# rokulkarni15/distributed-llm-training-inference

Measured on AMD Instinct MI355X. Metric: train tok/s Llama-2-7B ZeRO-3+LoRA at 1/2/4/8 GPUs; serve tok/s + p50 TTFT, higher is better.
Workload: dtype bf16

## Files before the change

### lumen/csrc/kernels/flash_attn.hip

```cpp
#include "common.h"
#include <cstdlib>

namespace lumen {
namespace fa {

typedef __bf16 bf16x8 __attribute__((ext_vector_type(8)));
typedef _Float16 f16x8 __attribute__((ext_vector_type(8)));
typedef float f32x4 __attribute__((ext_vector_type(4)));
typedef short s16x4 __attribute__((ext_vector_type(4)));
typedef __attribute__((address_space(3))) s16x4 lds_s16x4;

constexpr int D = 128;
constexpr int BN = 64;
constexpr int IMG = BN * D * 2;

template <typename T> struct Mfma;
template <> struct Mfma<bf16> {
  static __device__ __forceinline__ f32x4 run(uint4 a, uint4 b, f32x4 c) {
    return __builtin_amdgcn_mfma_f32_16x16x32_bf16(__builtin_bit_cast(bf16x8, a),
                                                   __builtin_bit_cast(bf16x8, b), c, 0, 0, 0);
  }
};
template <> struct Mfma<fp16> {
  static __device__ __forceinline__ f32x4 run(uint4 a, uint4 b, f32x4 c) {
    return __builtin_amdgcn_mfma_f32_16x16x32_f16(__builtin_bit_cast(f16x8, a),
                                                  __builtin_bit_cast(f16x8, b), c, 0, 0, 0);
  }
};

__device__ __forceinline__ int swz(int row) { return ((row & 3) << 2) | ((row >> 2) & 3); }
__device__ __forceinline__ int img_off(int row, int chunk) {
  return row * 256 + ((chunk ^ swz(row)) << 4);
}
template <int SW>
__device__ __forceinline__ int swz_t(int row) {
  if constexpr (SW == 0) return swz(row);
  else return ((row & 1) << 3) | ((row & 2) << 1) | ((row & 4) >> 1);
}
__device__ __forceinline__ unsigned lds_off_g(const char* p) {
  return static_cast<unsigned>(
      reinterpret_cast<uintptr_t>((__attribute__((address_space(3))) const char*)(p)));
}
template <int SW>
__device__ __forceinline__ int img_off_t(int row, int chunk) {
  return row * 256 + ((chunk ^ swz_t<SW>(row)) << 4);
}

template <typename T>
__device__ __forceinline__ void stage64(char* img, const T* base, long long ld, int r0, int rmax) {
#pragma unroll
  for (int i = 0; i < 4; ++i) {
    const int idx = threadIdx.x + i * 256;
    const int row = idx >> 4, ch = idx & 15;
    uint4 v = make_uint4(0, 0, 0, 0);
    if (r0 + row < rmax) v = *reinterpret_cast<const uint4*>(base + (long long)(r0 + row) * ld + ch * 8);
    *reinterpret_cast<uint4*>(img + img_off(row, ch)) = v;
  }
}

template <typename T, int SW = 0>
__device__ __forceinline__ void stage64_async(char* img, const T* base, long long ld, int r0,
                                              int rmax) {
  const int lane = threadIdx.x & 63, wid = threadIdx.x >> 6;
#pragma unroll
  for (int i = 0; i < 4; ++i) {
    const int row = (wid * 4 + i) * 4 + (lane >> 4);
    const int ch = (lane & 15) ^ swz_t<SW>(row);
    int gr = r0 + row;
    gr = gr < rmax ? gr : rmax - 1;
    __builtin_amdgcn_global_load_lds(
        (const void*)(base + (long long)gr * ld + ch * 8),
        (__attribute__((address_space(3))) void*)(img + (wid * 4 + i) * 1024), 16, 0, 0);
  }
}

template <typename T>
__device__ __forceinline__ void stage64_async_s(char* img, const T* base, long long ld, int r0,
                                                int rmax) {
  const int lane = threadIdx.x & 63, wid = __builtin_amdgcn_readfirstlane(threadIdx.x >> 6);
  const char* tile = reinterpret_cast<const char*>(base + (long long)r0 * ld);
  const int last = rmax - 1 - r0;
#pragma unroll
  for (int i = 0; i < 4; ++i) {
    const int row = (wid * 4 + i) * 4 + (lane >> 4);
    const int ch = (lane & 15) ^ swz(row);
    const unsigned off = (unsigned)((row < last ? row : last) * (int)ld + ch * 8) * sizeof(T);
    __builtin_amdgcn_global_load_lds(
        (const void*)(tile + off),
        (__attribute__((address_space(3))) void*)(img + (wid * 4 + i) * 1024), 16, 0, 0);
  }
}

__device__ __forceinline__ void dma16_o(const void* g, const char* lds_wave_base) {
  const unsigned m0 = __builtin_amdgcn_readfirstlane(lds_off_g(lds_wave_base));
  asm volatile("s_mov_b32 m0, %1\n\ts_nop 0\n\tglobal_load_lds_dwordx4 %0, off"
               :: "v"(g), "s"(m0) : "memory", "m0");
}
__device__ __forceinline__ void dma4_o(const void* g, const char* lds_wave_base) {
  const unsigned m0 = __builtin_amdgcn_readfirstlane(lds_off_g(lds_wave_base));
  asm volatile("s_mov_b32 m0, %1\n\ts_nop 0\n\tglobal_load_lds_dword %0, off"
               :: "v"(g), "s"(m0) : "memory", "m0");
}
template <typename T, int SW>
__device__ __forceinline__ void stage64_async_o(char* img, const T* base, long long ld, int r0,
                                                int rmax) {
  const int lane = threadIdx.x & 63, wid = __builtin_amdgcn_readfirstlane(threadIdx.x >> 6);
#pragma unroll
  for (int i = 0; i < 4; ++i) {
    const int row = (wid * 4 + i) * 4 + (lane >> 4);
    const int ch = (lane & 15) ^ swz_t<SW>(row);
    int gr = r0 + row;
    gr = gr < rmax ? gr : rmax - 1;
    dma16_o(base + (long long)gr * ld + ch * 8, img + (wid * 4 + i) * 1024);
  }
}

template <typename T, int SW>
__device__ __forceinline__ void stage64_async8_o(char* img, const T* base, long long ld, int r0,
                                                 int rmax) {
  const int lane = threadIdx.x & 63, wid = threadIdx.x >> 6;
#pragma unroll
  for (int i = 0; i < 2; ++i) {
    const int row = (wid * 2 + i) * 4 + (lane >> 4);
    const int ch = (lane & 15) ^ swz_t<SW>(row);
    int gr = r0 + row;
    gr = gr < rmax ? gr : rmax - 1;
    dma16_o(base + (long long)gr * ld + ch * 8, img + (wid * 2 + i) * 1024);
  }
}

template <typename T>
__device__ __forceinline__ void stage64_paged(char* img, const T* cache, int kvh, int nkv,
                                              const int* bt, int bs, int r0, int rmax) {
  const int lane = threadIdx.x & 63, wid = threadIdx.x >> 6;
#pragma unroll
  for (int i = 0; i < 4; ++i) {
    const int row = (wid * 4 + i) * 4 + (lane >> 4);
    const int ch = (lane & 15) ^ swz(row);
    int gr = r0 + row;
    gr = gr < rmax ? gr : rmax - 1;
    const long long blk = bt[gr / bs];
    const T* src = cache + ((blk * nkv + kvh) * bs + gr % bs) * D + ch * 8;
    __builtin_amdgcn_global_load_lds(
        (const void*)src, (__attribute__((address_space(3))) void*)(img + (wid * 4 + i) * 1024),
        16, 0, 0);
  }
}

__device__ __forceinline__ void wait_vm_all() { __builtin_amdgcn_s_waitcnt(0xF70); }
__device__ __forceinline__ void wait_vm_8() { __builtin_amdgcn_s_waitcnt(0xF78); }
__device__ __forceinline__ void lds_fence_barrier() {
  asm volatile("s_waitcnt lgkmcnt(0)" ::: "memory");
  __builtin_amdgcn_s_barrier();
  asm volatile("" ::: "memory");
}

template <int SW = 0>
__device__ __forceinline__ uint4 row_read(const char* img, int row, int chunk) {
  return *reinterpret_cast<const uint4*>(img + img_off_t<SW>(row, chunk));
}

__device__ __forceinline__ uint2 tr_read_raw(const char* p) {
  s16x4 r = __builtin_amdgcn_ds_read_tr16_b64_v4i16((lds_s16x4*)(p));
  return __builtin_bit_cast(uint2, r);
}

__device__ __forceinline__ uint4 tr_read_img(const char* img, int k0, int n0, int lane) {
  const int L = lane & 15, g = lane >> 4;
  const int col = n0 + 4 * (L & 3);
  const int ch = col >> 3, half = (col >> 2) & 1;
  const int r = k0 + 8 * g + (L >> 2);
  const uint2 lo = tr_read_raw(img + img_off(r, ch) + 8 * half);
  const uint2 hi = tr_read_raw(img + img_off(r + 4, ch) + 8 * half);
  return make_uint4(lo.x, lo.y, hi.x, hi.y);
}

__device__ __forceinline__ uint4 tr_read_y(const char* y, int cols, int k0, int m0, int lane) {
  const int L = lane & 15, g = lane >> 4;
  const int r = k0 + 8 * g + (L >> 2);
  const int c = m0 + 4 * (L & 3);
  const int ld = cols + 4;
  const uint2 lo = tr_read_raw(y + (r * ld + c) * 2);
  const uint2 hi = tr_read_raw(y + ((r + 4) * ld + c) * 2);
  return make_uint4(lo.x, lo.y, hi.x, hi.y);
}

template <typename T>
__device__ __forceinline__ void y_store(char* y, int cols, int k0, int m0, int lane, float v0,
                                        float v1, float v2, float v3) {
  T t[4] = {from_f32<T>(v0), from_f32<T>(v1), from_f32<T>(v2), from_f32<T>(v3)};
  *reinterpret_cast<uint2*>(y + ((k0 + (lane & 15)) * (cols + 4) + m0 + 4 * (lane >> 4)) * 2) =
      *reinterpret_cast<uint2*>(t);
}

template <typename T>
__device__ __forceinline__ uint4 gload16(const T* p, bool ok) {
  return ok ? *reinterpret_cast<const uint4*>(p) : make_uint4(0, 0, 0, 0);
}

template <int CTRL>
__device__ __forceinline__ float dpp(float v) {
  return __builtin_bit_cast(float, __builtin_amdgcn_update_dpp(0, __builtin_bit_cast(int, v), CTRL,
                                                               0xF, 0xF, false));
}
__device__ __forceinline__ float red16_max(float v) {
  v = fmaxf(v, dpp<0xB1>(v));
  v = fmaxf(v, dpp<0x4E>(v));
  v = fmaxf(v, dpp<0x141>(v));
  v = fmaxf(v, dpp<0x140>(v));
  return v;
}
__device__ __forceinline__ float red16_sum(float v) {
  v += dpp<0xB1>(v);
  v += dpp<0x4E>(v);
  v += dpp<0x141>(v);
  v += dpp<0x140>(v);
  return v;
}

__device__ __forceinline__ float fexp2(float x) { return __builtin_amdgcn_exp2f(x); }

struct Args {
  const void* q; const void* k; const void* v;
  long long ldq, ldk, ldv;
  void* o; long long ldo;
  float* lse;
  const int* cu;
  const int* tiles;
  int nh, nkv, T;
  float scale, scale_log2;
  const void* dout; long long lddo;
  void* dq; void* dk; void* dv; long long lddq, lddk, lddv;
  const float* delta;
  const int* rope_pos;
  const float* rope_cos;
  const float* rope_sin;
  const int* kv_lens;
  const int* block_tables;
// ... 910 lines not shown
```

### lumen/csrc/kernels/lora_v3.hip

```cpp
#include "tile128.h"
#include "det.h"

namespace lumen {
namespace lv3 {

using namespace tile;

struct Drop {
  unsigned int seed, thresh;
  float scale;
  long long ld;
  long long col0;
};

__device__ __forceinline__ uint4 mask8(uint4 u, uint32_t keep) {
  const auto wm = [keep](int w) {
    return ((keep >> (2 * w)) & 1u ? 0x0000FFFFu : 0u) | ((keep >> (2 * w + 1)) & 1u ? 0xFFFF0000u : 0u);
  };
  return make_uint4(u.x & wm(0), u.y & wm(1), u.z & wm(2), u.w & wm(3));
}

template <typename T>
__device__ __forceinline__ uint4 ld_f32x8(const float* p, bool ok) {
  if (!ok) return make_uint4(0, 0, 0, 0);
  const float4 u = *reinterpret_cast<const float4*>(p);
  const float4 v = *reinterpret_cast<const float4*>(p + 4);
  return make_uint4(pk2<T>(u.x, u.y), pk2<T>(u.z, u.w), pk2<T>(v.x, v.y), pk2<T>(v.z, v.w));
}

struct DownArgs {
  const void* x; long long ldx;
  const float* A; long long lda;
  float* Z; long long ldz;
  int T, K;
  float alpha;
  Drop drop;
  int probe;
  void* xe; long long ldxe; int xk, KP;
  unsigned* cnt;
  float* slab;
};

template <typename T, bool DROP, int NJ>
__global__ void __launch_bounds__(512) down3_kernel(DownArgs a) {
  constexpr int J = NJ * 16, JP = J + 4;
  __shared__ float red[4][64 * JP];
  const int wid = threadIdx.x >> 6, lane = threadIdx.x & 63, L = lane & 15, g = lane >> 4;
  const int t0 = blockIdx.x * 64;
  const int k0 = (blockIdx.y * 8 + wid) * 128;
  f32x4 acc[4][NJ];
#pragma unroll
  for (int rt = 0; rt < 4; ++rt)
#pragma unroll
    for (int jt = 0; jt < NJ; ++jt) acc[rt][jt] = f32x4{0.f, 0.f, 0.f, 0.f};
  if (k0 < a.K) {
    const T* x = reinterpret_cast<const T*>(a.x);
    uint4 xv[4][4];
#pragma unroll
    for (int rt = 0; rt < 4; ++rt)
#pragma unroll
      for (int i = 0; i < 4; ++i) {
        const int t = t0 + rt * 16 + L, c = k0 + 32 * i + 8 * g;
        xv[rt][i] = (t < a.T && c < a.K)
                        ? *reinterpret_cast<const uint4*>(x + (long long)t * a.ldx + c)
                        : make_uint4(0, 0, 0, 0);
      }
    float4 af[4][NJ][2];
    if (!(a.probe & 2)) {
#pragma unroll
      for (int i = 0; i < 4; ++i) {
        const int c = min(k0 + 32 * i + 8 * g, a.K - 8);
#pragma unroll
        for (int jt = 0; jt < NJ; ++jt) {
          const float* ap = a.A + (long long)(jt * 16 + L) * a.lda + c;
          af[i][jt][0] = *reinterpret_cast<const float4*>(ap);
          af[i][jt][1] = *reinterpret_cast<const float4*>(ap + 4);
        }
      }
    }
    if (DROP && !(a.probe & 1)) {
#pragma unroll
      for (int rt = 0; rt < 4; ++rt)
#pragma unroll
// ... 216 lines not shown
    if (rt + 1 < kUpRT && t0 + 16 < a.T) load_tile(t0 + 16, bnxt, ynxt);
    f32x4 acc[8];
#pragma unroll
    for (int n = 0; n < 8; ++n) acc[n] = f32x4{0.f, 0.f, 0.f, 0.f};
#pragma unroll
    for (int ks = 0; ks < NKS; ++ks)
#pragma unroll
      for (int n = 0; n < 8; ++n) acc[n] = Mfma<T>::run(aop[n][ks], bcur[ks], acc[n]);
    const int t = t0 + L;
    float y[4][8];
#pragma unroll
    for (int i = 0; i < 4; ++i) {
      unpack8<T>(ycur[i], y[i]);
      const int c = c0 + 32 * i + 8 * g;
      const uint32_t keep = DROP ? dropout_keep8(a.drop.seed,
                                                 (unsigned long long)((long long)t * a.drop.ld + a.drop.col0 + a.seg.out_off[seg] + c),
                                                 a.drop.thresh)
                                 : 0xFFu;
      const float sc = DROP ? a.alpha * a.drop.scale : a.alpha;
#pragma unroll
      for (int e = 0; e < 8; ++e) {
        const float d = acc[2 * i + (e >> 2)][e & 3];
        y[i][e] += ((keep >> e) & 1u) ? sc * d : 0.f;
      }
    }
    if (rope && t < a.T) {
      const long long p = (long long)a.rope_pos[t] * 64;
      float cs[2][8], sn[2][8];
#pragma unroll
      for (int h = 0; h < 2; ++h) {
        const float* cp = a.rope_cos + p + 32 * h + 8 * g;
        const float* sp = a.rope_sin + p + 32 * h + 8 * g;
        const float4 c_lo = *reinterpret_cast<const float4*>(cp), c_hi = *reinterpret_cast<const float4*>(cp + 4);
        const float4 s_lo = *reinterpret_cast<const float4*>(sp), s_hi = *reinterpret_cast<const float4*>(sp + 4);
        cs[h][0] = c_lo.x; cs[h][1] = c_lo.y; cs[h][2] = c_lo.z; cs[h][3] = c_lo.w;
        cs[h][4] = c_hi.x; cs[h][5] = c_hi.y; cs[h][6] = c_hi.z; cs[h][7] = c_hi.w;
        sn[h][0] = s_lo.x; sn[h][1] = s_lo.y; sn[h][2] = s_lo.z; sn[h][3] = s_lo.w;
        sn[h][4] = s_hi.x; sn[h][5] = s_hi.y; sn[h][6] = s_hi.z; sn[h][7] = s_hi.w;
      }
#pragma unroll
      for (int i = 0; i < 2; ++i)
#pragma unroll
        for (int e = 0; e < 8; ++e) {
          const float lo = y[i][e], hi = y[i + 2][e];
          y[i][e] = lo * cs[i][e] - hi * sn[i][e];
          y[i + 2][e] = hi * cs[i][e] + lo * sn[i][e];
        }
    }
    if (t < a.T) {
#pragma unroll
      for (int i = 0; i < 4; ++i) {
        const int c = c0 + 32 * i + 8 * g;
        if (c < NC) store8(out + (long long)t * a.ldo + c, y[i]);
      }
    }
#pragma unroll
    for (int ks = 0; ks < NKS; ++ks) bcur[ks] = bnxt[ks];
#pragma unroll
    for (int i = 0; i < 4; ++i) ycur[i] = ynxt[i];
  }
}

struct DySeg {
  long long n_off[4], r_off[4], b_off[4];
  int n_len[4];
  int nseg;
};

struct DyArgs {
  const void* dy; long long ldy;
  const float* B; int r;
  const float* Z; long long ldz;
  float* dZ; long long lddz;
  float* dB;
  int T, TW;
  float alpha;
  DySeg seg;
  int probe;
  float* slab_z; float* slab_b;
  unsigned* cnt_z; unsigned* cnt_b;
};

constexpr int kDyCC = 2;

template <typename T>
__device__ __forceinline__ void dy_load(uint4 (&v)[4], const T* base, long long ld, int r0, int rmax,
                                        int c0, int cmax) {
#pragma unroll
  for (int i = 0; i < 4; ++i) {
    const int idx = threadIdx.x + i * 256;
    const int r = r0 + (idx >> 4), c = c0 + (idx & 15) * 8;
    const uint4 u = *reinterpret_cast<const uint4*>(base + (long long)min(r, rmax - 1) * ld +
                                                     min(c, cmax - 8));
    v[i] = (r < rmax && c < cmax) ? u : make_uint4(0, 0, 0, 0);
  }
}

__device__ __forceinline__ void dy_store(char* img, const uint4 (&v)[4]) {
#pragma unroll
  for (int i = 0; i < 4; ++i) {
    const int idx = threadIdx.x + i * 256;
    *reinterpret_cast<uint4*>(img + img_off_b(idx >> 4, idx & 15)) = v[i];
  }
}

template <typename T, int NJ>
__global__ void __launch_bounds__(256) dy3_kernel(DyArgs a) {
  __shared__ __attribute__((aligned(16))) char img[2][64 * 256];
  const int seg = blockIdx.z;
  const int NL = a.seg.n_len[seg];
  const int cb = blockIdx.x * 128 * kDyCC;
  const int tb = blockIdx.y * a.TW, te = min(a.T, tb + a.TW);
  if (cb >= NL || tb >= a.T) return;
  const int lane = threadIdx.x & 63, wid = threadIdx.x >> 6, L = lane & 15, g = lane >> 4;
  const T* dy = reinterpret_cast<const T*>(a.dy) + a.seg.n_off[seg];
  const float* B = a.B + a.seg.b_off[seg] * a.r;
  const float* Z = a.Z + a.seg.r_off[seg];
  float* dZ = a.dZ + a.seg.r_off[seg];
  float* dB = a.dB + a.seg.b_off[seg] * a.r;
  const int nch = min(kDyCC, (NL - cb + 127) / 128);

  uint4 bop[kDyCC][4][NJ];
#pragma unroll
  for (int cc = 0; cc < kDyCC; ++cc)
#pragma unroll
    for (int i = 0; i < 4; ++i)
#pragma unroll
      for (int jt = 0; jt < NJ; ++jt) {
        float f[8];
#pragma unroll
        for (int e = 0; e < 8; ++e) {
          const int c = cb + cc * 128 + 32 * i + 8 * g + e;
          const float u = B[(long long)min(c, NL - 1) * a.r + jt * 16 + L];
          f[e] = c < NL ? u : 0.f;
        }
        bop[cc][i][jt] = pack8<T>(f);
      }
  f32x4 dbacc[kDyCC][2][NJ];
#pragma unroll
  for (int cc = 0; cc < kDyCC; ++cc)
#pragma unroll
    for (int m = 0; m < 2; ++m)
#pragma unroll
      for (int jt = 0; jt < NJ; ++jt) dbacc[cc][m][jt] = f32x4{0.f, 0.f, 0.f, 0.f};

  const int nsub = (te - tb + 63) / 64;
  const int nstage = nsub * nch;
  uint4 v[4];
  dy_load<T>(v, dy, a.ldy, tb, te, cb, NL);
  int buf = 0;
  f32x4 dzacc[NJ];
  uint4 zop[2][NJ];
  for (int s = 0; s < nstage; ++s, buf ^= 1) {
    const int ts = s / nch, cc = s % nch;
    const int t0 = tb + ts * 64, cbase = cb + cc * 128;
    dy_store(img[buf], v);
    __syncthreads();
    float zf[2][NJ][8];
#pragma unroll
    for (int ks = 0; ks < 2; ++ks)
#pragma unroll
      for (int jt = 0; jt < NJ; ++jt)
#pragma unroll
        for (int e = 0; e < 8; ++e) {
          const int t = t0 + 32 * ks + 8 * g + e;
          zf[ks][jt][e] = Z[(long long)min(t, te - 1) * a.ldz + jt * 16 + L];
        }
    {
      const int s1 = min(s + 1, nstage - 1);
      const int ts1 = s1 / nch, cc1 = s1 % nch;
      dy_load<T>(v, dy, a.ldy, tb + ts1 * 64, te, cb + cc1 * 128, NL);
    }
    if (cc == 0) {
#pragma unroll
      for (int jt = 0; jt < NJ; ++jt) dzacc[jt] = f32x4{0.f, 0.f, 0.f, 0.f};
    }
    const char* im = img[buf];
#pragma unroll
    for (int i = 0; i < 4; ++i) {
      const uint4 av = row_read_b(im, wid * 16 + L, i * 4 + g);
#pragma unroll
      for (int c2 = 0; c2 < kDyCC; ++c2)
        if (c2 == cc) {
#pragma unroll
          for (int jt = 0; jt < NJ; ++jt) dzacc[jt] = Mfma<T>::run(av, bop[c2][i][jt], dzacc[jt]);
        }
    }
#pragma unroll
    for (int ks = 0; ks < 2; ++ks)
#pragma unroll
      for (int jt = 0; jt < NJ; ++jt) {
        float f[8];
#pragma unroll
        for (int e = 0; e < 8; ++e) f[e] = t0 + 32 * ks + 8 * g + e < te ? zf[ks][jt][e] : 0.f;
        zop[ks][jt] = pack8<T>(f);
      }
#pragma unroll
    for (int ks = 0; ks < 2; ++ks)
#pragma unroll
      for (int m = 0; m < 2; ++m) {
        const uint4 tv = tr_read_img_b(im, ks * 32, wid * 32 + m * 16, lane);
#pragma unroll
        for (int c2 = 0; c2 < kDyCC; ++c2)
          if (c2 == cc) {
#pragma unroll
            for (int jt = 0; jt < NJ; ++jt) dbacc[c2][m][jt] = Mfma<T>::run(tv, zop[ks][jt], dbacc[c2][m][jt]);
          }
      }
    if (cc == nch - 1) {
      if (a.slab_z != nullptr) {
        float* sz = a.slab_z + (((long long)seg * gridDim.y + blockIdx.y) * gridDim.x + blockIdx.x) *
                                   ((long long)a.TW * a.r);
#pragma unroll
        for (int jt = 0; jt < NJ; ++jt)
#pragma unroll
          for (int r = 0; r < 4; ++r) {
            const int t = t0 + wid * 16 + g * 4 + r;
            if (t < te) det::st_wt(sz + (long long)(t - tb) * a.r + jt * 16 + L, dzacc[jt][r]);
          }
      } else {
#pragma unroll
        for (int jt = 0; jt < NJ; ++jt)
#pragma unroll
          for (int r = 0; r < 4; ++r) {
            const int t = t0 + wid * 16 + g * 4 + r;
            if (t < te && (!(a.probe & 16) || dzacc[jt][r] == 1234.5f))
              atomicAdd(dZ + (long long)t * a.lddz + jt * 16 + L, a.alpha * dzacc[jt][r]);
          }
      }
    }
  }
  if (a.slab_z != nullptr) {
    float* sb = a.slab_b + (((long long)seg * gridDim.x + blockIdx.x) * gridDim.y + blockIdx.y) *
                               (256LL * a.r);
#pragma unroll
    for (int cc = 0; cc < kDyCC; ++cc) {
      if (cc >= nch) break;
#pragma unroll
      for (int m = 0; m < 2; ++m)
#pragma unroll
        for (int jt = 0; jt < NJ; ++jt)
#pragma unroll
          for (int r = 0; r < 4; ++r) {
            const int cl = cc * 128 + wid * 32 + m * 16 + g * 4 + r;
            if (cb + cl < NL) det::st_wt(sb + (long long)cl * a.r + jt * 16 + L, dbacc[cc][m][jt][r]);
          }
    }
    if (a.cnt_z == nullptr) return;
    __shared__ int lastf;
    const int ncb = (NL + 128 * kDyCC - 1) / (128 * kDyCC);
    const int J = NJ * 16;
    if (det::last_arriver(a.cnt_z + (long long)seg * gridDim.y + blockIdx.y, ncb, &lastf)) {
      const float* base = a.slab_z + ((long long)seg * gridDim.y + blockIdx.y) * gridDim.x *
                                         ((long long)a.TW * a.r);
      for (int i = threadIdx.x; i < (te - tb) * (J / 2); i += 256) {
        const int tl = i / (J / 2), j = (i % (J / 2)) * 2;
        const float2 v = det::sum_pairs(base + (long long)tl * a.r + j, (long long)a.TW * a.r, ncb);
        float* o = dZ + (long long)(tb + tl) * a.lddz + j;
        o[0] = a.alpha * v.x;
        o[1] = a.alpha * v.y;
      }
    }
    if (det::last_arriver(a.cnt_b + (long long)seg * gridDim.x + blockIdx.x, gridDim.y, &lastf)) {
      const float* base = a.slab_b + ((long long)seg * gridDim.x + blockIdx.x) * gridDim.y *
                                         (256LL * a.r);
      const int nc = min(256, NL - cb);
      for (int i = threadIdx.x; i < nc * (J / 2); i += 256) {
        const int cl = i / (J / 2), j = (i % (J / 2)) * 2;
        const float2 v = det::sum_pairs(base + (long long)cl * a.r + j, 256LL * a.r, gridDim.y);
        float* o = dB + (long long)(cb + cl) * a.r + j;
        o[0] += a.alpha * v.x;
        o[1] += a.alpha * v.y;
      }
    }
    return;
  }
#pragma unroll
  for (int cc = 0; cc < kDyCC; ++cc) {
    if (cc >= nch) break;
#pragma unroll
    for (int m = 0; m < 2; ++m)
#pragma unroll
      for (int jt = 0; jt < NJ; ++jt) {
#pragma unroll
        for (int r = 0; r < 4; ++r) {
          const int c = cb + cc * 128 + wid * 32 + m * 16 + g * 4 + r;
          if (c < NL && (!(a.probe & 32) || dbacc[cc][m][jt][r] == 1234.5f))
            atomicAdd(dB + (long long)c * a.r + jt * 16 + L, a.alpha * dbacc[cc][m][jt][r]);
        }
      }
  }
}

__device__ __forceinline__ float2 sum_pairs_plain(const float* base, long long stride, int n) {
  float2 v = make_float2(0.f, 0.f);
  for (int q0 = 0; q0 < n; q0 += 16) {
    float2 u[16];
#pragma unroll
    for (int k = 0; k < 16; ++k) {
      const int q = q0 + k < n ? q0 + k : n - 1;
      u[k] = *reinterpret_cast<const float2*>(base + q * stride);
    }
#pragma unroll
    for (int k = 0; k < 16; ++k)
      if (q0 + k < n) {
        v.x += u[k].x;
        v.y += u[k].y;
      }
  }
  return v;
}

__global__ void __launch_bounds__(256) dy3_reduce_kernel(DyArgs a, int gx_n, int gy_n) {
  const int seg = blockIdx.y;
  const int NL = a.seg.n_len[seg];
  const int hr = a.r / 2;
  const long long i = (long long)blockIdx.x * 256 + threadIdx.x;
  const int j = (int)(i % hr) * 2;
  if (blockIdx.z == 0) {
    const long long t = i / hr;
    if (t >= a.T) return;
    const int gy = (int)(t / a.TW), tl = (int)(t % a.TW);
    const int ncb = (NL + 128 * kDyCC - 1) / (128 * kDyCC);
    const float* base = a.slab_z + (((long long)seg * gy_n + gy) * gx_n) * ((long long)a.TW * a.r) +
                        (long long)tl * a.r + j;
    const float2 v = sum_pairs_plain(base, (long long)a.TW * a.r, ncb);
    float* o = a.dZ + a.seg.r_off[seg] + t * a.lddz + j;
    o[0] = a.alpha * v.x;
    o[1] = a.alpha * v.y;
  } else {
    const long long c = i / hr;
    if (c >= NL) return;
    const int gx = (int)(c / (128 * kDyCC)), cl = (int)(c % (128 * kDyCC));
    const float* base = a.slab_b + (((long long)seg * gx_n + gx) * gy_n) * (256LL * a.r) +
                        (long long)cl * a.r + j;
    const float2 v = sum_pairs_plain(base, 256LL * a.r, gy_n);
    float* o = a.dB + (a.seg.b_off[seg] + c) * a.r + j;
    o[0] += a.alpha * v.x;
    o[1] += a.alpha * v.y;
  }
}

__global__ void __launch_bounds__(256) dxa3_reduce_kernel(const float* __restrict__ slab,
                                                          float* __restrict__ dA, long long ldda,
                                                          int R, int K, int gy_n, float scale) {
  const long long i = (long long)blockIdx.x * 256 + threadIdx.x;
// ... 378 lines not shown
    default: LV3_DOWN(TT, 4); break;                                                             \
  }
  if (dtype == kBF16) { LV3_DOWN_NJ(bf16) }
  else if (dtype == kF16) { LV3_DOWN_NJ(fp16) }
  else return hipErrorInvalidValue;
#undef LV3_DOWN_NJ
#undef LV3_DOWN
  if (slab != nullptr && cnt == nullptr) {
    const long long n = (long long)T * (R / 2);
    hipLaunchKernelGGL(lv3::down3_reduce_kernel, dim3((unsigned)((n + 255) / 256)), dim3(256), 0,
                       st, (const float*)slab, Z, ldz, T, R, (int)grid.y);
  }
  return hipGetLastError();
}

extern "C" hipError_t lumen_lora3_up(int dtype, int fwd, void* out, long long ldo, const float* s1,
                                     long long ld1, const float* s2, long long ld2, int T, int J,
                                     float alpha, unsigned long long seed, unsigned int thresh,
                                     float drop_scale, long long drop_ld, long long drop_col0,
                                     int nseg, const long long* out_off, const long long* s1_off,
                                     const long long* s2_off, const int* ncols,
                                     const float* rope_cos, const float* rope_sin,
                                     const int* rope_pos, int rope_mask, hipStream_t st) {
  if (T <= 0 || J < 1 || J > 64 || nseg < 1 || nseg > 4 || (ldo & 7) || (ld1 & 3) || (ld2 & 3))
    return hipErrorInvalidValue;
  lv3::UpArgs a;
  a.out = out; a.ldo = ldo; a.s1 = s1; a.ld1 = ld1; a.s2 = s2; a.ld2 = ld2; a.T = T; a.J = J;
  a.alpha = alpha;
  a.drop = {static_cast<unsigned>(seed) ^ static_cast<unsigned>(seed >> 32), thresh, drop_scale,
            drop_ld, drop_col0};
  a.seg.nseg = nseg;
  int maxc = 0;
  for (int i = 0; i < 4; ++i) {
    const bool v = i < nseg;
    a.seg.out_off[i] = v ? out_off[i] : 0; a.seg.s1_off[i] = v ? s1_off[i] : 0;
    a.seg.s2_off[i] = v ? s2_off[i] : 0; a.seg.ncols[i] = v ? ncols[i] : 0;
    if (v && ((ncols[i] & 7) || (out_off[i] & 7) || (s1_off[i] & 3))) return hipErrorInvalidValue;
    if (v && ncols[i] > maxc) maxc = ncols[i];
  }
  a.rope_cos = rope_cos; a.rope_sin = rope_sin; a.rope_pos = rope_pos;
  a.rope_mask = (fwd && rope_cos && rope_sin && rope_pos) ? rope_mask : 0;
  for (int i = 0; i < nseg; ++i)
    if (((a.rope_mask >> i) & 1) && ((out_off[i] & 127) || (ncols[i] & 127))) return hipErrorInvalidValue;
  if (maxc == 0) return hipSuccess;
  const dim3 grid((maxc + 127) / 128, (T + 64 * lv3::kUpRT - 1) / (64 * lv3::kUpRT), nseg), block(256);
  const bool drop = !fwd && thresh != 0;
#define LV3_UP(TT, KJ)                                                                             \
  do {                                                                                           \
    if (fwd) hipLaunchKernelGGL((lv3::up3_kernel<TT, true, false, KJ>), grid, block, 0, st, a);   \
    else if (drop) hipLaunchKernelGGL((lv3::up3_kernel<TT, false, true, KJ>), grid, block, 0, st, a); \
    else hipLaunchKernelGGL((lv3::up3_kernel<TT, false, false, KJ>), grid, block, 0, st, a);     \
  } while (0)
  if (dtype == kBF16) { if (J <= 32) LV3_UP(bf16, 32); else LV3_UP(bf16, 64); }
  else if (dtype == kF16) { if (J <= 32) LV3_UP(fp16, 32); else LV3_UP(fp16, 64); }
  else return hipErrorInvalidValue;
#undef LV3_UP
  return hipGetLastError();
}

extern "C" hipError_t lumen_lora3_dy(int dtype, const void* dy, long long ldy, const float* B, int r,
                                     const float* Z, long long ldz, float* dZ, long long lddz,
                                     float* dB, int T, int tw, float alpha, int nseg,
                                     const long long* n_off, const long long* r_off,
                                     const long long* b_off, const int* n_len, float* slab_z,
                                     float* slab_b, unsigned* cnt_z, unsigned* cnt_b,
                                     hipStream_t st) {
  if (T <= 0 || nseg < 1 || nseg > 4 || (r != 16 && r != 32 && r != 64) || tw < 64 || (tw & 63) ||
      (ldy & 7))
    return hipErrorInvalidValue;
  lv3::DyArgs a;
  a.probe = lv3_probe();
  a.dy = dy; a.ldy = ldy; a.B = B; a.r = r; a.Z = Z; a.ldz = ldz; a.dZ = dZ; a.lddz = lddz;
  a.dB = dB; a.T = T; a.TW = tw; a.alpha = alpha;
  a.slab_z = slab_z; a.slab_b = slab_b; a.cnt_z = cnt_z; a.cnt_b = cnt_b;
  if (slab_z != nullptr && (slab_b == nullptr || (cnt_z == nullptr) != (cnt_b == nullptr) ||
                            (lddz & 1)))
    return hipErrorInvalidValue;
  a.seg.nseg = nseg;
  int maxl = 0;
  for (int i = 0; i < 4; ++i) {
    const bool v = i < nseg;
    a.seg.n_off[i] = v ? n_off[i] : 0; a.seg.r_off[i] = v ? r_off[i] : 0;
    a.seg.b_off[i] = v ? b_off[i] : 0; a.seg.n_len[i] = v ? n_len[i] : 0;
    if (v && ((n_len[i] & 7) || (n_off[i] & 7))) return hipErrorInvalidValue;
    if (v && n_len[i] > maxl) maxl = n_len[i];
  }
  if (maxl == 0) return hipSuccess;
  const dim3 grid((maxl + 128 * lv3::kDyCC - 1) / (128 * lv3::kDyCC), (T + tw - 1) / tw, nseg), block(256);
#define LV3_DY(TT)                                                                                 \
  switch (r) {                                                                                   \
    case 16: hipLaunchKernelGGL((lv3::dy3_kernel<TT, 1>), grid, block, 0, st, a); break;          \
    case 32: hipLaunchKernelGGL((lv3::dy3_kernel<TT, 2>), grid, block, 0, st, a); break;          \
    default: hipLaunchKernelGGL((lv3::dy3_kernel<TT, 4>), grid, block, 0, st, a); break;          \
  }
  if (dtype == kBF16) { LV3_DY(bf16) }
  else if (dtype == kF16) { LV3_DY(fp16) }
  else return hipErrorInvalidValue;
#undef LV3_DY
  if (slab_z != nullptr && cnt_z == nullptr) {
    const long long n = (long long)(T > maxl ? T : maxl) * (r / 2);
    const dim3 rgrid((unsigned)((n + 255) / 256), nseg, 2);
    hipLaunchKernelGGL(lv3::dy3_reduce_kernel, rgrid, dim3(256), 0, st, a, (int)grid.x,
                       (int)grid.y);
  }
  return hipGetLastError();
}

extern "C" hipError_t lumen_lora3_z_tail(int dtype, const float* Z, int R, void* xe, long long ldx,
                                         int K, int KP, int T, hipStream_t st) {
  if (T <= 0) return hipSuccess;
  if ((KP & 7) || R > KP || (ldx & 7) || (K & 7)) return hipErrorInvalidValue;
  const long long n = static_cast<long long>(T) * (KP / 8);
  const dim3 grid(static_cast<unsigned>((n + 255) / 256)), block(256);
  if (dtype == kBF16) hipLaunchKernelGGL(lv3::z_tail_kernel<bf16>, grid, block, 0, st, Z, R, (bf16*)xe, ldx, K, KP, T);
  else if (dtype == kF16) hipLaunchKernelGGL(lv3::z_tail_kernel<fp16>, grid, block, 0, st, Z, R, (fp16*)xe, ldx, K, KP, T);
  else return hipErrorInvalidValue;
  return hipGetLastError();
}

extern "C" hipError_t lumen_lora3_w_tail(int dtype, void* w, long long ldw, int K, const float* B,
                                         int r, int nseg, const long long* n_off,
                                         const long long* b_off, const int* n_len,
                                         const int* r_off, float scale, hipStream_t st) {
  if (nseg < 1 || nseg > 4 || (r & 7) || (ldw & 7) || (K & 7)) return hipErrorInvalidValue;
  lv3::TailSeg sg;
  sg.nseg = nseg;
  int maxn = 0;
  for (int i = 0; i < 4; ++i) {
    const bool v = i < nseg;
    sg.n_off[i] = v ? n_off[i] : 0; sg.b_off[i] = v ? b_off[i] : 0;
    sg.n_len[i] = v ? n_len[i] : 0; sg.r_off[i] = v ? r_off[i] : 0;
    if (v && (r_off[i] & 7)) return hipErrorInvalidValue;
    if (v && n_len[i] > maxn) maxn = n_len[i];
  }
  if (maxn == 0) return hipSuccess;
  const long long n = static_cast<long long>(maxn) * (r / 8);
  const dim3 grid(static_cast<unsigned>((n + 255) / 256), nseg), block(256);
  if (dtype == kBF16) hipLaunchKernelGGL(lv3::w_tail_kernel<bf16>, grid, block, 0, st, (bf16*)w, ldw, K, B, r, sg, scale);
  else if (dtype == kF16) hipLaunchKernelGGL(lv3::w_tail_kernel<fp16>, grid, block, 0, st, (fp16*)w, ldw, K, B, r, sg, scale);
  else return hipErrorInvalidValue;
  return hipGetLastError();
}

extern "C" hipError_t lumen_lora3_dxa(int dtype, const void* x, long long ldx, void* dx,
                                      long long lddx, const float* dZ, const float* A,
                                      long long lda, float* dA, long long ldda, int T, int K,
                                      int R, int tw, unsigned long long seed, unsigned int thresh,
                                      float drop_scale, long long drop_ld, long long drop_col0,
                                      float* delta, float* slab, unsigned* cnt, hipStream_t st) {
  if (T <= 0 || K <= 0 || R < 16 || R > 64 || (R & 15) || (K & 7) || (ldx & 7) || (lddx & 7) ||
      (lda & 3) || tw < 64 || (tw & 63))
    return hipErrorInvalidValue;
  if (delta != nullptr && ((K & 127) || R != 16)) return hipErrorInvalidValue;
  lv3::DxaArgs a;
  a.probe = lv3_probe();
  a.x = x; a.ldx = ldx; a.dx = dx; a.lddx = lddx; a.dZ = dZ; a.A = A; a.lda = lda; a.dA = dA;
  a.ldda = ldda; a.T = T; a.K = K; a.R = R; a.TW = tw; a.delta = delta;
  a.slab = slab; a.cnt = cnt;
  if (slab != nullptr && (ldda & 1)) return hipErrorInvalidValue;
  const bool drop = thresh != 0;
  a.da_scale = drop ? drop_scale : 1.f;
  a.dx_scale = drop ? drop_scale : 1.f;
  a.drop = {static_cast<unsigned>(seed) ^ static_cast<unsigned>(seed >> 32), thresh, drop_scale,
            drop_ld, drop_col0};
  const dim3 grid((K + 127) / 128, (T + tw - 1) / tw), block(256);
#define LV3_DXA(TT, NJ)                                                                            \
  do {                                                                                           \
    if (drop) hipLaunchKernelGGL((lv3::dxa3_kernel<TT, true, NJ>), grid, block, 0, st, a);      \
    else hipLaunchKernelGGL((lv3::dxa3_kernel<TT, false, NJ>), grid, block, 0, st, a);          \
// ... 31 lines not shown
```

### lumen/ops/lora.py

```python
from __future__ import annotations

import math
from typing import List, Optional, Sequence, Tuple

import torch
import torch.nn.functional as F

from ._native import DTYPE_CODE, native, use_native
from .gemm import mm_nt

Seg = Tuple[int, int, int, int]

_M32 = 0xFFFFFFFF


def _lowbias32(x):
    x = x ^ (x >> 16)
    x = (x * 0x7FEB352D) & _M32
    x = x ^ (x >> 15)
    x = (x * 0x846CA68B) & _M32
    x = x ^ (x >> 16)
    return x


# ... 108 lines not shown


def arena_reset(device) -> None:
    if USE_ARENA and device.type == "cuda":
        ARENA.reset(device)


def _zeros(*shape, device, train: bool = False):
    if USE_ARENA and device.type == "cuda" and (train or _IN_BACKWARD[0]):
        return ARENA.zeros(*shape, device=device)
    return torch.zeros(*shape, device=device, dtype=torch.float32)


USE_V3 = _os.environ.get("LUMEN_LORA_V3", "1") != "0"
DY_TW = int(_os.environ.get("LUMEN_LORA_DY_TW", "0"))
DXA_TW = int(_os.environ.get("LUMEN_LORA_DXA_TW", "0"))
DET_SPLIT = _os.environ.get("LUMEN_DET_SPLIT", "1") != "0"
DXA = _os.environ.get("LUMEN_LORA_DXA", "1") != "0"
DELTA_HANDOFF = _os.environ.get("LUMEN_FA_DELTA_HANDOFF", "1") != "0"
_DELTA_SLOT = [None]


DETERMINISTIC = _os.environ.get("LUMEN_LORA_DETERMINISTIC", "0") == "1"
_det: dict = {}


def _det_ws(dev, nfloat: int, ncnt: int):
    key = (str(dev), torch.cuda.current_stream(dev).cuda_stream)
    got = _det.get(key)
    if got is None or got[0].numel() < nfloat or got[1].numel() < ncnt:
        nf = max(nfloat, got[0].numel() if got is not None else 0, 1 << 20)
        nc = max(ncnt, got[1].numel() if got is not None else 0, 4096)
        got = (torch.empty(nf, dtype=torch.float32, device=dev),
               torch.zeros(nc, dtype=torch.int32, device=dev))
        _det[key] = got
    return got


def _v3_ok(r: int, R: int, segs, *mats) -> bool:
    return (USE_V3 and r in (16, 32, 64) and R % 16 == 0 and R <= 64
            and all(s[0] % 8 == 0 and s[1] % 8 == 0 for s in segs)
            and all(m.stride(1) == 1 and m.stride(0) % 8 == 0 for m in mats))


def _lora3_down(x2d, A, Z, p, seed):
    T, K = x2d.shape
    R = A.shape[0]
    cnt = slab = None
    if DETERMINISTIC and x2d.is_cuda:
        slab, cnt = _det_ws(x2d.device, math.ceil(T / 64) * math.ceil(K / 1024) * 64 * R,
                            math.ceil(T / 64))
    native().lora3_down(x2d, x2d.stride(0), A, Z, R, T, K, R, 1.0, int(seed) & 0x7FFFFFFFFFFFFFFF,
                        drop_threshold(p), 1.0 / (1.0 - p) if p > 0 else 1.0, K, 0,
                        None, 0, 0, None if (slab is not None and DET_SPLIT) else cnt, slab)


def _lora3_fwd(x2d, y, A, B, Z, segs, r, scale, p, seed, rope):
    _lora3_down(x2d, A, Z, p, seed)
    fuse = rope is not None and len(segs) <= 4 and _rope_covered(segs, rope[3])
    for i in range(0, len(segs), 4):
        ch = segs[i:i + 4]
        mask = sum(1 << j for j, sg in enumerate(ch) if sg[0] + sg[1] <= rope[3]) if fuse else 0
        _lora2(2, 1, B, Z, y, y.stride(0), 1, scale, T=x2d.shape[0], J=r, split=1,
               segs4=[(b_off * r, r_off, n_off, n_len) for (n_off, n_len, r_off, b_off) in ch],
               rope=(rope[1], rope[2], rope[0], mask) if fuse else None)
    return y, fuse


FOLD = _os.environ.get("LUMEN_LORA_FOLD", "1") != "0"
FOLD_KP = 64


def fold_operand(x2d: torch.Tensor, K: int) -> Optional[torch.Tensor]:
    if (x2d.dim() == 2 and x2d.shape[1] == K and x2d.stride(1) == 1
            and x2d.stride(0) == K + FOLD_KP and x2d.is_cuda):
        return x2d.as_strided((x2d.shape[0], K + FOLD_KP), (K + FOLD_KP, 1))
    return None


def _dy_tw(segs, T: int) -> int:
    if DY_TW:
        return DY_TW
    cols = sum(math.ceil(s[1] / 256) for s in segs)
    return 256 if cols * math.ceil(T / 256) >= 512 else 128


def lora_fwd_native(x2d, y, A, B, segs: Sequence[Seg], r, scale, p, seed, train: bool = False,
                    rope=None):
    T, K = x2d.shape
    R = A.shape[0]
    v3 = (_v3_ok(r, R, segs, x2d, y) and K % 8 == 0
          and A.is_contiguous() and B.is_contiguous() and A.dtype == B.dtype == torch.float32)
    Ntot = y.shape[1]
    act = DTYPE_CODE[x2d.dtype]
    Z = _zeros(T, R, device=x2d.device, train=train)
    if v3:
        y, fuse = _lora3_fwd(x2d, y, A, B, Z, segs, r, scale, p, seed, rope)
        return Z, fuse
    if _v2_ok(r, R, x2d):
        _lora2(0, 1, x2d, A, Z, R, 1, 1.0, T, R, _split(math.ceil(T / 64), K, 256),
               [(0, 0, 0, K)], seed, p, K)
    else:
        _lora_gemm(act, 1, x2d, A, Z, K, K, R, 1, 1.0, [(0, 0, 0, T, R, K)],
                   _ksplit(T, R, K, _bn(R)), seed, p, K)
    if _v2_ok(r, R, x2d, y) and all(s[0] % 8 == 0 and s[1] % 8 == 0 for s in segs):
        fuse = rope is not None and len(segs) <= 4 and _rope_covered(segs, rope[3])
        for i in range(0, len(segs), 4):
            ch = segs[i:i + 4]
            rp = None
            if fuse:
                mask = sum(1 << j for j, sg in enumerate(ch) if sg[0] + sg[1] <= rope[3])
                rp = (rope[1], rope[2], rope[0], mask)
            _lora2(2, 1, B, Z, y, y.stride(0), 1, scale, T, r, 1,
                   [(b_off * r, r_off, n_off, n_len) for (n_off, n_len, r_off, b_off) in ch],
                   rope=rp)
        return Z, fuse
    segs6 = [(r_off, b_off * r, n_off, T, n_len, r) for (n_off, n_len, r_off, b_off) in segs]
    for i in range(0, len(segs6), 4):
        _lora_gemm(act, 6, Z, B, y, R, r, Ntot, 1, scale, segs6[i:i + 4], 1)
    return Z, False


def _rope_covered(segs, ncols: int) -> bool:
    cov = sorted((s[0], s[0] + s[1]) for s in segs if s[0] < ncols)
    cur = 0
    for a, b in cov:
        if a != cur or b > ncols or a % 128 or b % 128:
            return False
        cur = b
    return cur == ncols


def lora_bwd_native(dy, x2d, A, B, Z, dx, segs: Sequence[Seg], r, scale, p, seed,
                    need_dA=True, need_dB=True, dx_fn=None):
    T, K = x2d.shape
    R = A.shape[0]
    Ntot = dy.shape[1]
    act = DTYPE_CODE[dy.dtype]
    dev = dy.device
    v2 = _v2_ok(r, R, x2d, dy)
    v3 = (v2 and _v3_ok(r, R, segs, x2d, dy) and K % 8 == 0 and A.is_contiguous()
          and B.is_contiguous() and A.dtype == B.dtype == torch.float32)
    v3 = v3 and (dx is None or _v3_ok(r, R, segs, dx))
    direct = v2 and DIRECT_GRAD and _direct_ok(A) and _direct_ok(B)
    if v3:
        return _lora3_bwd(dy, x2d, A, B, Z, dx, segs, r, scale, p, seed, need_dA, need_dB, direct,
                          dx_fn)
    if dx_fn is not None:
        dx = dx_fn()
    nA = R * K if need_dA and not direct else 0
    nB = B.shape[0] * r if need_dB and not direct else 0
    ws = _zeros(T * R + nA + nB, device=dev)
    dZ = ws[:T * R].view(T, R)
    if v2:
        for i in range(0, len(segs), 4):
            ch = segs[i:i + 4]
            _lora2(0, 0, dy, B, dZ, R, 1, scale, T, r,
                   _split(math.ceil(T / 64) * len(ch), max(s[1] for s in ch), 256),
                   [(n_off, b_off * r, r_off, n_len) for (n_off, n_len, r_off, b_off) in ch])
    else:
        s2 = [(n_off, b_off * r, r_off, T, r, n_len) for (n_off, n_len, r_off, b_off) in segs]
        for i in range(0, len(s2), 4):
            chunk = s2[i:i + 4]
            _lora_gemm(act, 2, dy, B, dZ, Ntot, r, R, 1, scale, chunk,
                       _ksplit(T, r, max(s[5] for s in chunk), 16, len(chunk)))
    dA = dB = None
    if need_dA:
# ... 302 lines not shown
```

Baseline: 45680.

## Pipeline LoRA dY kernel with LDS DMA ring and staged Z/B transposes

Rewrites the LoRA backward dy3 kernel to stage dY tiles through a 4-deep LDS ring filled by global_load_lds DMA with vmcnt-based waits, replacing the register double buffer. Z and B are now loaded with vectorized float4 reads, packed into a swizzled transposed LDS buffer once per 512-row superblock, and read back as MFMA operands, instead of scalar per-element gathers on every stage. The token-window heuristic is widened to pick tiles of up to 512 rows while keeping at least a minimum block count. Shared DMA helpers move into a common header and now save and restore m0. The larger LDS footprint may lower occupancy, and new alignment checks reject some inputs.

```diff
diff --git a/lumen/csrc/kernels/flash_attn.hip b/lumen/csrc/kernels/flash_attn.hip
--- a/lumen/csrc/kernels/flash_attn.hip
+++ b/lumen/csrc/kernels/flash_attn.hip
@@ -1,8 +1,14 @@
 #include "common.h"
+#include "lds_dma.h"
 #include <cstdlib>
 
 namespace lumen {
 namespace fa {
+
+using tile::dma16_o;
+using tile::dma4_o;
+using tile::lds_fence_barrier;
+using tile::lds_off_g;
 
 typedef __bf16 bf16x8 __attribute__((ext_vector_type(8)));
 typedef _Float16 f16x8 __attribute__((ext_vector_type(8)));
@@ -36,10 +42,6 @@
 __device__ __forceinline__ int swz_t(int row) {
   if constexpr (SW == 0) return swz(row);
   else return ((row & 1) << 3) | ((row & 2) << 1) | ((row & 4) >> 1);
-}
-__device__ __forceinline__ unsigned lds_off_g(const char* p) {
-  return static_cast<unsigned>(
-      reinterpret_cast<uintptr_t>((__attribute__((address_space(3))) const char*)(p)));
 }
 template <int SW>
 __device__ __forceinline__ int img_off_t(int row, int chunk) {
@@ -91,16 +93,6 @@
   }
 }
 
-__device__ __forceinline__ void dma16_o(const void* g, const char* lds_wave_base) {
-  const unsigned m0 = __builtin_amdgcn_readfirstlane(lds_off_g(lds_wave_base));
-  asm volatile("s_mov_b32 m0, %1\n\ts_nop 0\n\tglobal_load_lds_dwordx4 %0, off"
-               :: "v"(g), "s"(m0) : "memory", "m0");
-}
-__device__ __forceinline__ void dma4_o(const void* g, const char* lds_wave_base) {
-  const unsigned m0 = __builtin_amdgcn_readfirstlane(lds_off_g(lds_wave_base));
-  asm volatile("s_mov_b32 m0, %1\n\ts_nop 0\n\tglobal_load_lds_dword %0, off"
-               :: "v"(g), "s"(m0) : "memory", "m0");
-}
 template <typename T, int SW>
 __device__ __forceinline__ void stage64_async_o(char* img, const T* base, long long ld, int r0,
                                                 int rmax) {
@@ -149,11 +141,6 @@
 
 __device__ __forceinline__ void wait_vm_all() { __builtin_amdgcn_s_waitcnt(0xF70); }
 __device__ __forceinline__ void wait_vm_8() { __builtin_amdgcn_s_waitcnt(0xF78); }
-__device__ __forceinline__ void lds_fence_barrier() {
-  asm volatile("s_waitcnt lgkmcnt(0)" ::: "memory");
-  __builtin_amdgcn_s_barrier();
-  asm volatile("" ::: "memory");
-}
 
 template <int SW = 0>
 __device__ __forceinline__ uint4 row_read(const char* img, int row, int chunk) {
diff --git a/lumen/csrc/kernels/lds_dma.h b/lumen/csrc/kernels/lds_dma.h
--- /dev/null
+++ b/lumen/csrc/kernels/lds_dma.h
@@ -0,0 +1,40 @@
+#pragma once
+#include "common.h"
+
+namespace lumen {
+namespace tile {
+
+__device__ __forceinline__ unsigned lds_off_g(const char* p) {
+  return static_cast<unsigned>(
+      reinterpret_cast<uintptr_t>((__attribute__((address_space(3))) const char*)(p)));
+}
+
+__device__ __forceinline__ void dma16_o(const void* g, const char* lds_wave_base) {
+  const unsigned m0 = __builtin_amdgcn_readfirstlane(lds_off_g(lds_wave_base));
+  unsigned keep;
+  asm volatile("s_mov_b32 %0, m0\n\ts_mov_b32 m0, %2\n\ts_nop 0\n\t"
+               "global_load_lds_dwordx4 %1, off\n\ts_mov_b32 m0, %0"
+               : "=&s"(keep) : "v"(g), "s"(m0) : "memory");
+}
+__device__ __forceinline__ void dma4_o(const void* g, const char* lds_wave_base) {
+  const unsigned m0 = __builtin_amdgcn_readfirstlane(lds_off_g(lds_wave_base));
+  unsigned keep;
+  asm volatile("s_mov_b32 %0, m0\n\ts_mov_b32 m0, %2\n\ts_nop 0\n\t"
+               "global_load_lds_dword %1, off\n\ts_mov_b32 m0, %0"
+               : "=&s"(keep) : "v"(g), "s"(m0) : "memory");
+}
+
+template <int N>
+__device__ __forceinline__ void wait_vm() {
+  static_assert(N >= 0 && N <= 63, "vmcnt is a 6-bit counter");
+  asm volatile("s_waitcnt vmcnt(%0)" :: "n"(N) : "memory");
+}
+
+__device__ __forceinline__ void lds_fence_barrier() {
+  asm volatile("s_waitcnt lgkmcnt(0)" ::: "memory");
+  __builtin_amdgcn_s_barrier();
+  asm volatile("" ::: "memory");
+}
+
+}
+}
diff --git a/lumen/csrc/kernels/lora_v3.hip b/lumen/csrc/kernels/lora_v3.hip
--- a/lumen/csrc/kernels/lora_v3.hip
+++ b/lumen/csrc/kernels/lora_v3.hip
@@ -1,4 +1,5 @@
 #include "tile128.h"
+#include "lds_dma.h"
 #include "det.h"
 
 namespace lumen {
@@ -381,37 +382,38 @@
 };
 
 constexpr int kDyCC = 2;
+constexpr int kDyRing = 4;
+constexpr int kDySB = 512;
+
+__device__ __forceinline__ int dy_zt_off(int j, int col) {
+  return j * kDySB + ((((col >> 3) ^ j) & 15) << 3 | (col & ~127)) + (col & 7);
+}
 
 template <typename T>
-__device__ __forceinline__ void dy_load(uint4 (&v)[4], const T* base, long long ld, int r0, int rmax,
-                                        int c0, int cmax) {
+__device__ __forceinline__ void dy_stage(char* img, const T* base, long long ld, int r0, int rmax,
+                                         int c0, int cmax) {
+  const int lane = threadIdx.x & 63, wid = __builtin_amdgcn_readfirstlane(threadIdx.x >> 6);
 #pragma unroll
   for (int i = 0; i < 4; ++i) {
-    const int idx = threadIdx.x + i * 256;
-    const int r = r0 + (idx >> 4), c = c0 + (idx & 15) * 8;
-    const uint4 u = *reinterpret_cast<const uint4*>(base + (long long)min(r, rmax - 1) * ld +
-                                                     min(c, cmax - 8));
-    v[i] = (r < rmax && c < cmax) ? u : make_uint4(0, 0, 0, 0);
-  }
-}
-
-__device__ __forceinline__ void dy_store(char* img, const uint4 (&v)[4]) {
-#pragma unroll
-  for (int i = 0; i < 4; ++i) {
-    const int idx = threadIdx.x + i * 256;
-    *reinterpret_cast<uint4*>(img + img_off_b(idx >> 4, idx & 15)) = v[i];
+    const int row = (wid * 4 + i) * 4 + (lane >> 4);
+    const int ch = (lane & 15) ^ swz_b(row);
+    dma16_o(base + (long long)min(r0 + row, rmax - 1) * ld + min(c0 + ch * 8, cmax - 8),
+            img + (wid * 4 + i) * 1024);
   }
 }
 
 template <typename T, int NJ>
 __global__ void __launch_bounds__(256) dy3_kernel(DyArgs a) {
-  __shared__ __attribute__((aligned(16))) char img[2][64 * 256];
+  constexpr int J = NJ * 16;
+  __shared__ __attribute__((aligned(16))) char ring[kDyRing][64 * 256];
+  __shared__ __attribute__((aligned(16))) T zt[J * kDySB];
   const int seg = blockIdx.z;
   const int NL = a.seg.n_len[seg];
   const int cb = blockIdx.x * 128 * kDyCC;
   const int tb = blockIdx.y * a.TW, te = min(a.T, tb + a.TW);
   if (cb >= NL || tb >= a.T) return;
   const int lane = threadIdx.x & 63, wid = threadIdx.x >> 6, L = lane & 15, g = lane >> 4;
+  static_assert(kDySB == 512 && kDyCC * 128 <= kDySB, "dy_zt_off swizzles within 128-column groups");
   const T* dy = reinterpret_cast<const T*>(a.dy) + a.seg.n_off[seg];
   const float* B = a.B + a.seg.b_off[seg] * a.r;
   const float* Z = a.Z + a.seg.r_off[seg];
@@ -419,92 +421,132 @@
   float* dB = a.dB + a.seg.b_off[seg] * a.r;
   const int nch = min(kDyCC, (NL - cb + 127) / 128);
 
+  const int sh = nch - 1;
+  const auto stage = [&](int s, int sb0, int se) {
+    dy_stage<T>(ring[s % kDyRing], dy, a.ldy, sb0 + (s >> sh) * 64, se, cb + (s & sh) * 128, NL);
+  };
+  constexpr int NI = J / 8;
+  float4 zf[NI][2];
+  const auto load_z = [&](int r0, int se) {
+#pragma unroll
+    for (int q = 0; q < NI; ++q) {
+      const int idx = threadIdx.x + q * 256, t = r0 + 2 * (idx / (J / 4)), j = (idx % (J / 4)) * 4;
+      zf[q][0] = *reinterpret_cast<const float4*>(Z + (long long)min(t, se - 1) * a.ldz + j);
+      zf[q][1] = *reinterpret_cast<const float4*>(Z + (long long)min(t + 1, se - 1) * a.ldz + j);
+    }
+  };
+  const auto store_pairs = [&](const float4 (&f)[NI][2], int q, int col0, bool ok0, bool ok1) {
+    const int idx = threadIdx.x + q * 256, p = idx / (J / 4), j = (idx % (J / 4)) * 4;
+    const float4 z = make_float4(0.f, 0.f, 0.f, 0.f);
+    const float4 u = ok0 ? f[q][0] : z, v = ok1 ? f[q][1] : z;
+    const int c = col0 + 2 * p;
+    *reinterpret_cast<unsigned*>(zt + dy_zt_off(j, c)) = pk2<T>(u.x, v.x);
+    *reinterpret_cast<unsigned*>(zt + dy_zt_off(j + 1, c)) = pk2<T>(u.y, v.y);
+    *reinterpret_cast<unsigned*>(zt + dy_zt_off(j + 2, c)) = pk2<T>(u.z, v.z);
+    *reinterpret_cast<unsigned*>(zt + dy_zt_off(j + 3, c)) = pk2<T>(u.w, v.w);
+  };
+  const auto store_z = [&](int r0, int sb0, int se) {
+#pragma unroll
+    for (int q = 0; q < NI; ++q) {
+      const int t = r0 + 2 * ((threadIdx.x + q * 256) / (J / 4));
+      store_pairs(zf, q, r0 - sb0, t < se, t + 1 < se);
+    }
+  };
+  {
+    const int se = min(te, tb + kDySB), ns = ((se - tb + 63) / 64) << sh;
+#pragma unroll
+    for (int s = 0; s < kDyRing - 1; ++s)
+      if (s < ns) stage(s, tb, se);
+    load_z(tb, se);
+  }
   uint4 bop[kDyCC][4][NJ];
+  {
+    float4 bf[NI][2];
+#pragma unroll
+    for (int q = 0; q < NI; ++q) {
+      const int idx = threadIdx.x + q * 256, c = cb + 2 * (idx / (J / 4)), j = (idx % (J / 4)) * 4;
+      bf[q][0] = *reinterpret_cast<const float4*>(B + (long long)min(c, NL - 1) * a.r + j);
+      bf[q][1] = *reinterpret_cast<const float4*>(B + (long long)min(c + 1, NL - 1) * a.r + j);
+    }
+#pragma unroll
+    for (int q = 0; q < NI; ++q) {
+      const int c = cb + 2 * ((threadIdx.x + q * 256) / (J / 4));
+      store_pairs(bf, q, 0, c < NL, c + 1 < NL);
+    }
+    lds_fence_barrier();
+#pragma unroll
+    for (int cc = 0; cc < kDyCC; ++cc)
+#pragma unroll
+      for (int i = 0; i < 4; ++i)
+#pragma unroll
+        for (int jt = 0; jt < NJ; ++jt)
+          bop[cc][i][jt] = *reinterpret_cast<const uint4*>(
+              zt + dy_zt_off(jt * 16 + L, cc * 128 + 32 * i + 8 * g));
+  }
+  f32x4 dbacc[kDyCC][2][NJ];
 #pragma unroll
   for (int cc = 0; cc < kDyCC; ++cc)
 #pragma unroll
-    for (int i = 0; i < 4; ++i)
-#pragma unroll
-      for (int jt = 0; jt < NJ; ++jt) {
-        float f[8];
-#pragma unroll
-        for (int e = 0; e < 8; ++e) {
-          const int c = cb + cc * 128 + 32 * i + 8 * g + e;
-          const float u = B[(long long)min(c, NL - 1) * a.r + jt * 16 + L];
-          f[e] = c < NL ? u : 0.f;
-        }
-        bop[cc][i][jt] = pack8<T>(f);
-      }
-  f32x4 dbacc[kDyCC][2][NJ];
-#pragma unroll
-  for (int cc = 0; cc < kDyCC; ++cc)
-#pragma unroll
     for (int m = 0; m < 2; ++m)
 #pragma unroll
       for (int jt = 0; jt < NJ; ++jt) dbacc[cc][m][jt] = f32x4{0.f, 0.f, 0.f, 0.f};
 
-  const int nsub = (te - tb + 63) / 64;
-  const int nstage = nsub * nch;
-  uint4 v[4];
-  dy_load<T>(v, dy, a.ldy, tb, te, cb, NL);
-  int buf = 0;
   f32x4 dzacc[NJ];
   uint4 zop[2][NJ];
-  for (int s = 0; s < nstage; ++s, buf ^= 1) {
-    const int ts = s / nch, cc = s % nch;
-    const int t0 = tb + ts * 64, cbase = cb + cc * 128;
-    dy_store(img[buf], v);
-    __syncthreads();
-    float zf[2][NJ][8];
-#pragma unroll
-    for (int ks = 0; ks < 2; ++ks)
-#pragma unroll
-      for (int jt = 0; jt < NJ; ++jt)
-#pragma unroll
-        for (int e = 0; e < 8; ++e) {
-          const int t = t0 + 32 * ks + 8 * g + e;
-          zf[ks][jt][e] = Z[(long long)min(t, te - 1) * a.ldz + jt * 16 + L];
-        }
-    {
-      const int s1 = min(s + 1, nstage - 1);
-      const int ts1 = s1 / nch, cc1 = s1 % nch;
-      dy_load<T>(v, dy, a.ldy, tb + ts1 * 64, te, cb + cc1 * 128, NL);
-    }
+  for (int sb0 = tb; sb0 < te; sb0 += kDySB) {
+  const int se = min(te, sb0 + kDySB);
+  const int nstage = ((se - sb0 + 63) / 64) << sh;
+  if (sb0 != tb) {
+    lds_fence_barrier();
+#pragma unroll
+    for (int s = 0; s < kDyRing - 1; ++s)
+      if (s < nstage) stage(s, sb0, se);
+    load_z(sb0, se);
+  } else {
+    lds_fence_barrier();
+  }
+  store_z(sb0, sb0, se);
+  if (se - sb0 > 256) {
+    load_z(sb0 + 256, se);
+    store_z(sb0 + 256, sb0, se);
+  }
+  for (int ts = 0; ts << sh < nstage; ++ts) {
+#pragma unroll
+  for (int cc = 0; cc < kDyCC; ++cc) {
+    if (cc >= nch) break;
+    const int s = (ts << sh) + cc;
+    const int t0 = sb0 + ts * 64;
+    static_assert(kDyRing == 4, "the waits below count two stages behind the one being read");
+    const int left = nstage - 1 - s;
+    if (left >= kDyRing - 2) wait_vm<4 * (kDyRing - 2)>();
+    else if (left == 1) wait_vm<4>();
+    else wait_vm<0>();
+    lds_fence_barrier();
+    if (s + kDyRing - 1 < nstage) stage(s + kDyRing - 1, sb0, se);
     if (cc == 0) {
 #pragma unroll
       for (int jt = 0; jt < NJ; ++jt) dzacc[jt] = f32x4{0.f, 0.f, 0.f, 0.f};
     }
-    const char* im = img[buf];
+    const char* im = ring[s % kDyRing];
 #pragma unroll
     for (int i = 0; i < 4; ++i) {
       const uint4 av = row_read_b(im, wid * 16 + L, i * 4 + g);
 #pragma unroll
-      for (int c2 = 0; c2 < kDyCC; ++c2)
-        if (c2 == cc) {
-#pragma unroll
-          for (int jt = 0; jt < NJ; ++jt) dzacc[jt] = Mfma<T>::run(av, bop[c2][i][jt], dzacc[jt]);
-        }
+      for (int jt = 0; jt < NJ; ++jt) dzacc[jt] = Mfma<T>::run(av, bop[cc][i][jt], dzacc[jt]);
     }
 #pragma unroll
     for (int ks = 0; ks < 2; ++ks)
 #pragma unroll
-      for (int jt = 0; jt < NJ; ++jt) {
-        float f[8];
-#pragma unroll
-        for (int e = 0; e < 8; ++e) f[e] = t0 + 32 * ks + 8 * g + e < te ? zf[ks][jt][e] : 0.f;
-        zop[ks][jt] = pack8<T>(f);
-      }
+      for (int jt = 0; jt < NJ; ++jt)
+        zop[ks][jt] = *reinterpret_cast<const uint4*>(
+            zt + dy_zt_off(jt * 16 + L, (t0 - sb0) + 32 * ks + 8 * g));
 #pragma unroll
     for (int ks = 0; ks < 2; ++ks)
 #pragma unroll
       for (int m = 0; m < 2; ++m) {
         const uint4 tv = tr_read_img_b(im, ks * 32, wid * 32 + m * 16, lane);
 #pragma unroll
-        for (int c2 = 0; c2 < kDyCC; ++c2)
-          if (c2 == cc) {
-#pragma unroll
-            for (int jt = 0; jt < NJ; ++jt) dbacc[c2][m][jt] = Mfma<T>::run(tv, zop[ks][jt], dbacc[c2][m][jt]);
-          }
+        for (int jt = 0; jt < NJ; ++jt) dbacc[cc][m][jt] = Mfma<T>::run(tv, zop[ks][jt], dbacc[cc][m][jt]);
       }
     if (cc == nch - 1) {
       if (a.slab_z != nullptr) {
@@ -529,6 +571,8 @@
       }
     }
   }
+  }
+  }
   if (a.slab_z != nullptr) {
     float* sb = a.slab_b + (((long long)seg * gridDim.x + blockIdx.x) * gridDim.y + blockIdx.y) *
                                (256LL * a.r);
@@ -546,10 +590,9 @@
           }
     }
     if (a.cnt_z == nullptr) return;
-    __shared__ int lastf;
+    int* lastf = reinterpret_cast<int*>(&ring[0][0]);
     const int ncb = (NL + 128 * kDyCC - 1) / (128 * kDyCC);
-    const int J = NJ * 16;
-    if (det::last_arriver(a.cnt_z + (long long)seg * gridDim.y + blockIdx.y, ncb, &lastf)) {
+    if (det::last_arriver(a.cnt_z + (long long)seg * gridDim.y + blockIdx.y, ncb, lastf)) {
       const float* base = a.slab_z + ((long long)seg * gridDim.y + blockIdx.y) * gridDim.x *
                                          ((long long)a.TW * a.r);
       for (int i = threadIdx.x; i < (te - tb) * (J / 2); i += 256) {
@@ -560,7 +603,7 @@
         o[1] = a.alpha * v.y;
       }
     }
-    if (det::last_arriver(a.cnt_b + (long long)seg * gridDim.x + blockIdx.x, gridDim.y, &lastf)) {
+    if (det::last_arriver(a.cnt_b + (long long)seg * gridDim.x + blockIdx.x, gridDim.y, lastf)) {
       const float* base = a.slab_b + ((long long)seg * gridDim.x + blockIdx.x) * gridDim.y *
                                          (256LL * a.r);
       const int nc = min(256, NL - cb);
@@ -1105,9 +1148,10 @@
     const bool v = i < nseg;
     a.seg.n_off[i] = v ? n_off[i] : 0; a.seg.r_off[i] = v ? r_off[i] : 0;
     a.seg.b_off[i] = v ? b_off[i] : 0; a.seg.n_len[i] = v ? n_len[i] : 0;
-    if (v && ((n_len[i] & 7) || (n_off[i] & 7))) return hipErrorInvalidValue;
+    if (v && ((n_len[i] & 7) || (n_off[i] & 7) || (r_off[i] & 3))) return hipErrorInvalidValue;
     if (v && n_len[i] > maxl) maxl = n_len[i];
   }
+  if (ldz & 3) return hipErrorInvalidValue;
   if (maxl == 0) return hipSuccess;
   const dim3 grid((maxl + 128 * lv3::kDyCC - 1) / (128 * lv3::kDyCC), (T + tw - 1) / tw, nseg), block(256);
 #define LV3_DY(TT)                                                                                 \
diff --git a/lumen/ops/lora.py b/lumen/ops/lora.py
--- a/lumen/ops/lora.py
+++ b/lumen/ops/lora.py
@@ -214,7 +214,13 @@
     if DY_TW:
         return DY_TW
     cols = sum(math.ceil(s[1] / 256) for s in segs)
-    return 256 if cols * math.ceil(T / 256) >= 512 else 128
+    for tw in range(512, 128, -64):
+        if cols * math.ceil(T / tw) >= _DY_MIN_BLOCKS:
+            return tw
+    return 128
+
+
+_DY_MIN_BLOCKS = 176
 
 
 def lora_fwd_native(x2d, y, A, B, segs: Sequence[Seg], r, scale, p, seed, train: bool = False,
```

Measured after the change: 45900 (median of 6 runs). No clear change (+0.5%).
